# google/FluidNet

Hardware: NVIDIA H100
Metric: sim steps/sec on 128^3 MAC grid (CNN proj) (higher is better)
Workload: dtype f32

## Files before the change

### fluidnet_b200/csrc/tfl_api.cu

```cuda
#include <string.h>
#include <algorithm>
#include <cmath>
#include <string>
#include <vector>

#include "tfl_api_internal.h"

namespace {

void widen_for_forward_pass(const tfl_ctx* ctx, const Geo& g, Geo* gf) {
  if (!ctx->slab) { gf->zlo = 0; gf->zhi = g.nz; return; }
  const int lo_lim = (g.zoff == 0) ? 0 : 1;
  const int hi_lim = (g.zoff + g.nz == g.gnz) ? g.nz : g.nz - 1;
  gf->zlo = std::max(lo_lim, g.zlo - ctx->slab_margin);
  gf->zhi = std::min(hi_lim, g.zhi + ctx->slab_margin);
}

int flag_cache_ensure(tfl_ctx* ctx, const Geo& g) {
  auto& fc = ctx->fcache;
  const size_t cells = (size_t)g.n * g.nb;
  if (!fc.changed) {
    void* p = nullptr;
    TFL_CUDA(ctx, cudaMalloc(&p, sizeof(int)));
    fc.changed = (int*)p;
// ... 739 lines not shown

int tfl_debug_advect_tile(tfl_ctx* ctx, int mode, int variant) {
  if (!ctx) return 1;
  ctx->tile.mode = mode;
  ctx->tile.variant = variant;
  return 0;
}

int tfl_debug_time_advect_kernel(tfl_ctx* ctx, int on) {
  if (!ctx) return 1;
  DeviceGuard guard_(ctx);
  auto& tl = ctx->tile;
  if (on && !tl.ev0) { cudaEventCreate(&tl.ev0); cudaEventCreate(&tl.ev1); }
  tl.timed = on != 0 && tl.ev0 && tl.ev1;
  return 0;
}
float tfl_debug_last_advect_kernel_ms(tfl_ctx* ctx) {
  if (!ctx || !ctx->tile.ev0) return -1.0f;
  DeviceGuard guard_(ctx);
  float ms = -1.0f;
  if (cudaEventSynchronize(ctx->tile.ev1) != cudaSuccess || cudaEventElapsedTime(&ms, ctx->tile.ev0, ctx->tile.ev1) != cudaSuccess) {
    cudaGetLastError();
    return -1.0f;
  }
  return ms;
}

static int set_const_vals(tfl_ctx* ctx, const tfl_state* s) {
  if (s->p_bc.data && s->p_bc_inv_mask.data && tfl_apply_bc(ctx, &s->p, &s->p_bc_inv_mask, &s->p_bc)) return 1;
  if (s->U_bc.data && s->U_bc_inv_mask.data && tfl_apply_bc(ctx, &s->U, &s->U_bc_inv_mask, &s->U_bc)) return 1;
  if (s->density.data && s->density_bc.data && s->density_bc_inv_mask.data &&
      tfl_apply_bc(ctx, &s->density, &s->density_bc_inv_mask, &s->density_bc))
    return 1;
  return 0;
}

static int simulate_step_fused(tfl_ctx* ctx, const tfl_state* s, const tfl_mconf* mc, tfl_cnn* m, const Geo& g) {
  const size_t cells = (size_t)g.n * g.nb;
  const bool has_density = s->density.data != nullptr;
  if (cnn_ensure_act(ctx, m, g)) return 1;
  if (arena_reserve(ctx, carve_bytes({cells * 4, cells * 4 * g.nc, cells * 4, cells * 4 * g.nc, cells * 4 * g.nc,
                                      cells * 12, cells * 4, cells * 4, 4 * (size_t)g.nb, cells * 12, cells / 4 + 64})))
    return 1;
  Carver cv(ctx);
  float* fwd_s = cv.take<float>(cells);
  float* fwd_pos = cv.take<float>(cells * g.nc);
  float* tmp_s = cv.take<float>(cells);
  float* fwd_u = cv.take<float>(cells * g.nc);
  float* tmp_u = cv.take<float>(cells * g.nc);
  float* curl = cv.take<float>(cells * 3);
  float* cnorm = cv.take<float>(cells);
  float* p_net = cv.take<float>(cells);
  float* scale = cv.take<float>(g.nb);
  float* force = cv.take<float>(cells * 3);
  unsigned char* qmask_buf = cv.take<unsigned char>(cells / 4 + 64);
  cudaStream_t st = ctx->stream;
  unsigned char *fl8 = nullptr, *clear = nullptr;
  if (prepare_flags(ctx, s->flags.data, g, &fl8, &clear)) return 1;
  const bool ov = ctx->ov.active;
  if (ov) TFL_CUDA(ctx, cudaStreamWaitEvent(st, ctx->ev_u_in, 0));
  const unsigned char* qmask = nullptr;
  const bool u_bc0 = s->U_bc.data && s->U_bc_inv_mask.data;
  const bool d_bc0 = has_density && s->density_bc.data && s->density_bc_inv_mask.data;
  bool qmask_on_side = false;
  if (has_density) {
    TFL_CUDA(ctx, cudaEventRecord(ctx->ev_fork, st));
// ... 29 lines not shown
  const bool u_bc = s->U_bc.data && s->U_bc_inv_mask.data;
  const bool d_bc = has_density && s->density_bc.data && s->density_bc_inv_mask.data;
  float bs[3] = {0.0f, 0.0f, 0.0f};
  const int do_buoy = has_density && fo.buoyancy;
  if (do_buoy)
    for (int a = 0; a < 3; a++) bs[a] = (-fo.buoy[a]) * scale_dt;
  launch_post_advect(has_density ? tmp_s : nullptr, tmp_u, fl8, has_density ? s->density.data : nullptr,
                     s->U.data, u_bc ? s->U_bc_inv_mask.data : nullptr, u_bc ? s->U_bc.data : nullptr,
                     d_bc ? s->density_bc_inv_mask.data : nullptr, d_bc ? s->density_bc.data : nullptr, qmask, do_buoy, bs,
                     g, st);
  ctx->launches += 1;
  if (ov && has_density && ctx->ov.density_host) {
    TFL_CUDA(ctx, cudaEventRecord(ctx->ev_d_ready, st));
    TFL_CUDA(ctx, cudaStreamWaitEvent(ctx->copy_out, ctx->ev_d_ready, 0));
    TFL_CUDA(ctx, cudaMemcpyAsync(ctx->ov.density_host, s->density.data, ctx->ov.density_bytes, cudaMemcpyDeviceToHost,
                                  ctx->copy_out));
    TFL_CUDA(ctx, cudaEventRecord(ctx->ev_d_out, ctx->copy_out));
    ctx->ov.density_sent = true;
  }
  if (fo.gravity) {
    const float f[3] = {fo.grav[0] * scale_dt, fo.grav[1] * scale_dt, fo.grav[2] * scale_dt};
    launch_add_gravity(s->U.data, fl8, f, g, st);
    ctx->launches += 1;
  }
  if (fo.vorticity) {
    launch_vort_curl(s->U.data, curl, cnorm, force, fo.vort_amp, g, st);
    ctx->launches += 2;
  }
  double* sums = ctx->dscratch + 64;
  TFL_CUDA(ctx, cudaMemsetAsync(sums, 0, sizeof(double) * 2 * g.nb, st));
  launch_vort_bc_mask(s->U.data, fl8, force, fo.vorticity, u_bc ? s->U_bc_inv_mask.data : nullptr,
                      u_bc ? s->U_bc.data : nullptr, qmask, 1, sums, g, st);
  const ConvTcGeo& tg = m->act_geo;
  if (ov) TFL_CUDA(ctx, cudaStreamWaitEvent(st, ctx->ev_p_in, 0));
  launch_cnn_inputs_fused(s->p.data, s->U.data, fl8, sums, mc->normalize_input_threshold, scale, m->act[0].get(),
                          tg.px, tg.py, g, st);
  run_conv_stack(m, p_net, st);
  launch_cnn_finish_fused(p_net, s->U.data, fl8, scale, s->p.data, u_bc ? s->U_bc_inv_mask.data : nullptr,
                          u_bc ? s->U_bc.data : nullptr, qmask, -1e6f, 1e6f, g, st);
  ctx->launches += 6;
  return check_launch(ctx, "simulate_step (fused)");
}

static bool fused_step_applies(const tfl_ctx* ctx, const tfl_state* s, const tfl_mconf* mc, const tfl_cnn* cnn) {
  return mc->sim_method == TFL_SIM_CONVNET && cnn && cnn->tc_ok && cnn->mode > 0 && cnn->default_inputs && !ctx->slab &&
         s->flags.nb == 1 &&
         !s->p_bc.data && mc->advection_method >= 0 && mc->advection_method <= 5;
}

int tfl_simulate_step(tfl_ctx* ctx, const tfl_state* s, const tfl_mconf* mc, tfl_cnn* cnn) {
  DeviceGuard guard_(ctx);
  NvtxRange range_(__func__);
  if (!s || !mc) return fail(ctx, "simulate: nil state / mconf");
  if (check_scalar(ctx, &s->flags, "flags") || check_scalar(ctx, &s->p, "pDiv") || check_vel(ctx, &s->U, &s->flags))
    return 1;
  const int is3d = s->U.nc == 3;
  Geo g;
  if (make_geo(ctx, &s->flags, is3d, &g)) return 1;
  const bool has_density = s->density.data != nullptr;
  if (fused_step_applies(ctx, s, mc, cnn)) {
    if (has_density && (check_scalar(ctx, &s->density, "density") || !same_spatial(&s->density, &s->flags)))
      return fail(ctx, "Size mismatch");
    return simulate_step_fused(ctx, s, mc, cnn, g);
  }
  if (has_density && tfl_advect_scalar(ctx, mc->dt, &s->density, &s->U, &s->flags, mc->advection_method, 0,
                                       mc->maccormack_strength, nullptr))
    return 1;
  if (tfl_advect_vel(ctx, mc->dt, &s->U, &s->flags, mc->advection_method, mc->maccormack_strength, nullptr))
    return 1;
  if (set_const_vals(ctx, s)) return 1;
  const StepForces fo = step_forces(mc, g.nx, g.ny, g.gnz);
  if (has_density && fo.buoyancy && tfl_add_buoyancy(ctx, &s->U, &s->flags, &s->density, fo.buoy, mc->dt))
    return 1;
// ... 192 lines not shown
```

### fluidnet_b200/csrc/tfl_api_cnn.cu

```cuda
#include <string.h>
#include <algorithm>
#include <cmath>
#include <vector>

#include "tfl_api_internal.h"

constexpr int kMaxBanks = kMaxBankPtrs;
constexpr char kSlabTcOnly[] =
    "the z-slab projection runs on the tensor-core path only (the 3-D 'default' graph, single-bank or with banks "
    "split at stage 1 and joined at stage 3, in mode 1 or 2)";
constexpr char kSlabDilate[] =
    "the z-slab projection does not run banksType 'dilate' (dilated banks run on whole grids only)";
constexpr char kSlabBatchNorm[] =
    "the z-slab projection does not run batch normalization (addBatchNorm models run on whole grids only)";
constexpr char kSlabDefaultInputs[] =
    "the z-slab projection takes the default input block only (inputChannels pDiv, div, flags; normalizeInput with "
    "'std' of UDiv; no addPressureSkip)";

constexpr int kTailFloats = 64 + 8 + 8 + 1;

namespace {

template <typename T>
DevPtr<T> dev_alloc(size_t n) {
// ... 205 lines not shown
    org[i] = m->borg[i - 1];
    float* dst = m->bact[3 * (i - 1)].get();
    if (m->bank_dilate) {
      launch_tc_phase_copy(in[0], tg, dst, geo[i], i, m->tc_planes, st);
    } else {
      launch_tc_pyramid(in[i - 1], geo[i - 1], dst, geo[i], org[i - 1] & 1, st, m->tc_planes);
    }
    in[i] = dst;
  }
  for (int i = 0; i < nbk; i++) {
    float* o1 = i == 0 ? m->act[1].get() : m->bact[3 * (i - 1) + 1].get();
    float* o2 = i == 0 ? m->act[2].get() : m->bact[3 * (i - 1) + 2].get();
    ConvTcGeo g1 = geo[i], g2 = geo[i];
    if (!m->bank_dilate) {
      const int c_lo = ((zoff + p_lo - 1) >> i) - org[i], c_hi = ((zoff + p_hi) >> i) - org[i] + 1;
      g2.z_lo = std::max(0, c_lo);     g2.z_hi = std::min(geo[i].nz, c_hi);
      g1.z_lo = std::max(0, c_lo - 1); g1.z_hi = std::min(geo[i].nz, c_hi + 1);
    }
    launch_conv3_tc(in[i], o1, nullptr, m->wBk[split][2 * i].get(), m->b[m->conv0[0] + i].get(), nullptr,
                    m->tc_planes, 0, split, g1, st, act);
    if (m->bank_dilate && i > 0 && ((tg.nx | tg.ny | tg.nz) & ((1 << i) - 1)))
      launch_tc_phase_zero(o1, geo[i], i, tg, st);
    launch_conv3_tc(o1, o2, nullptr, m->wBk[split][2 * i + 1].get(), m->b[m->conv0[1] + i].get(), nullptr, 2, 0,
                    split, g2, st, act);
    l2[i] = o2;
  }
  ConvTcGeo g3 = tg;
  g3.z_lo = std::max(0, p_lo);
  g3.z_hi = std::min(tg.nz, p_hi);
  launch_tc_join(l2, geo, org, zoff, nbk, m->bank_add, m->part.get(), p_net, m->wBj[split], m->b[m->conv0[2]].get(),
                 m->tail.get(), split, g3, st, m->bank_dilate != 0, act);
}

void run_conv_stack(tfl_cnn* m, float* p_net, cudaStream_t st, int p_lo, int p_hi) {
  if (p_hi < 0) p_hi = m->act_geo.nz;
  if (m->nbanks > 1) {
    run_conv_stack_banked(m, p_net, st, p_lo, p_hi);
    return;
  }
  const ConvTcGeo& tg = m->act_geo;
  const int split = m->mode == 2 ? 1 : 0;
  ConvTcGeo g1 = tg, g2 = tg, g3 = tg;
  g3.z_lo = std::max(0, p_lo);     g3.z_hi = std::min(tg.nz, p_hi);
  g2.z_lo = std::max(0, p_lo - 1); g2.z_hi = std::min(tg.nz, p_hi + 1);
  g1.z_lo = std::max(0, p_lo - 2); g1.z_hi = std::min(tg.nz, p_hi + 2);
  TcEpi e1, e2, e3;
  e1.relu6 = e2.relu6 = e3.relu6 = m->nonlin == 3;
  if (m->bn && !m->bn_batch) {
    e1.ac = m->bn_ac[0].get();
    e2.ac = m->bn_ac[1].get();
  }
  float *a0 = m->act[0].get(), *a1 = m->act[1].get(), *a2 = m->act[2].get(), *tail = m->tail.get();
  const float *w1 = m->wBk[split][0].get(), *w2 = m->wBk[split][1].get(), *w3 = m->wBj[split][0].get();
  if (!m->bn_batch) {
    launch_conv3_tc(a0, a1, nullptr, w1, m->b[0].get(), nullptr, m->tc_planes, 0, split, g1, st, e1);
    launch_conv3_tc(a1, a2, nullptr, w2, m->b[1].get(), nullptr, 2, 0, split, g2, st, e2);
    launch_conv3_tc(a2, nullptr, p_net, w3, m->b[2].get(), tail, 2, 1, split, g3, st, e3);
    return;
  }
  double* part = m->bn_part.get();
  float* ac = m->bn_tcac.get();
  const long long count = (long long)tg.nb * tg.nz * tg.ny * tg.nx;
  auto stats = [&](const float* buf, int l) {
    launch_tc_bn_stats(buf, tg, part, st);
    const float* wb = m->bn_wb[l].get();
    launch_bn_finalize(part, 8, count, wb, wb + 8, m->bn_eps[l], ac + 16 * l, nullptr, st);
  };
  launch_conv3_tc(a0, a1, nullptr, w1, m->b[0].get(), nullptr, m->tc_planes, 0, split, tg, st, e1);
  stats(a1, 0);
  launch_tc_bn_apply(a1, tg, ac, st);
  launch_conv3_tc(a1, a2, nullptr, w2, m->b[1].get(), nullptr, 2, 0, split, tg, st, e2);
  stats(a2, 1);
  launch_tc_bn_apply(a2, tg, ac + 16, st);
  launch_conv3_tc(a2, a1, nullptr, w3, m->b[2].get(), nullptr, 2, 0, split, tg, st, e3);
  stats(a1, 2);
  launch_tc_bn_tail(a1, tg, ac + 32, tail, e3.relu6, 0, part, nullptr, nullptr, st);
  launch_bn_finalize(part, 8, count, m->bn_wb[3].get(), m->bn_wb[3].get() + 8, m->bn_eps[3], ac + 48, nullptr, st);
  launch_tc_bn_tail(a1, tg, ac + 32, tail, e3.relu6, 1, nullptr, ac + 48, p_net, st);
}

static const tfl_cnn_inputs kDefaultInputs = {1, 0, 1, 1, 0, 0, 0};

namespace {

struct CnnSpec {
  int is_3d, n_layers;
  const int32_t *cin, *cout, *ksize, *pool, *up;
  int pool_is_max, nonlin_sigmoid;
// ... 960 lines not shown
```

### fluidnet_b200/csrc/tfl_api_internal.h

```cpp
#pragma once
#include <cuda_runtime.h>
#include <stdarg.h>
#include <stdio.h>
#include <nvtx3/nvToolsExt.h>
#include <nccl.h>
#include <initializer_list>
#include <memory>
#include <string>
#include <vector>

#include "tfl_kernels.h"
#include "tfl_cnn_tc.h"

using namespace tfl;

struct CudaFree {
  void operator()(void* p) const { cudaFree(p); }
};
template <typename T>
using DevPtr = std::unique_ptr<T, CudaFree>;

constexpr char kConvZStalled[] =
    "internal error, the z-streaming tensor-core convolution's pipeline stalled (a bounded wait ran out)";

// ... 169 lines not shown
  if (U->nc != 2 && U->nc != 3) return fail(ctx, "2D velocity field must have only 2 channels");
  if (U->nc == 2 && flags->nz != 1) return fail(ctx, "2D velocity field but zdepth > 1");
  if (!same_spatial(U, flags)) return fail(ctx, "Size mismatch");
  return 0;
}

inline int make_geo(tfl_ctx* ctx, const tfl_grid* flags, int is3d, Geo* g) {
  g->nx = flags->nx; g->ny = flags->ny; g->nz = flags->nz; g->nb = flags->nb;
  g->is3d = is3d ? 1 : 0;
  g->nc = is3d ? 3 : 2;
  g->n = (long long)flags->nx * flags->ny * flags->nz;
  g->faults = ctx->counters;
  if (ctx->slab) {
    if (!is3d) return fail(ctx, "slab decomposition needs a 3D grid");
    g->zoff = ctx->zoff; g->gnz = ctx->gnz; g->zlo = ctx->zlo; g->zhi = ctx->zhi;
    if (g->zlo < 0 || g->zhi > g->nz || g->zlo >= g->zhi || g->zoff < 0 || g->zoff + g->nz > g->gnz)
      return fail(ctx, "slab range does not fit the local grid");
  } else {
    g->zoff = 0; g->gnz = flags->nz; g->zlo = 0; g->zhi = flags->nz;
  }
  if (!is3d && flags->nz != 1) return fail(ctx, "2D grid must have zsize == 1");
  if (g->n >= (1LL << 31) || g->n * (long long)g->nb * 3 >= (1LL << 31) * 4) return fail(ctx, "grid too large");
  return 0;
}

struct StepForces {
  bool buoyancy, gravity, vorticity;
  float buoy[3], grav[3];
  float vort_amp;
};
StepForces step_forces(const tfl_mconf* mc, int nx, int ny, int gnz);

int cnn_ensure_act(tfl_ctx* ctx, tfl_cnn* m, const Geo& g);
void run_conv_stack(tfl_cnn* m, float* p_net, cudaStream_t st, int p_lo = 0, int p_hi = -1);
int cnn_slab_check(tfl_ctx* ctx, const tfl_cnn* m, int margin, int gnz, int ny, int nx, int zoff, int nz, int own_lo,
                   int own_hi);
```

### fluidnet_b200/csrc/tfl_cnn_tc.cu

```cuda
#include <cuda_runtime.h>
#include <stdint.h>

#include "tfl_cnn_tc.h"

namespace tfl {

namespace {

constexpr int kTX = 32;
constexpr int kGroups = 9;
constexpr int kThreads = 256;
constexpr int kDPitch = 24;

template <bool SPLIT> struct Tile {
  static constexpr int TY = SPLIT ? 4 : 8;
  static constexpr int TZ = SPLIT ? 5 : 6;
  static constexpr int PY = TY + 2, PZ = TZ + 2;
  static constexpr int RB = TY / 2;
  static constexpr int POS = kTX * PY * PZ;
  static constexpr int PLANE_BYTES = POS * 16;
  static constexpr int MTILES = TZ * RB;
};

template <int IN_PLANES, bool SPLIT> struct Layout {
  using T = Tile<SPLIT>;
  static constexpr int NB = SPLIT ? 48 : 32;
  static constexpr int GROUPS = IN_PLANES == 1 ? 5 : kGroups;
  static constexpr int ZERO_BYTES = IN_PLANES == 1 ? 64 * 16 : 0;
  static constexpr int PSTRIDE = T::PLANE_BYTES + ZERO_BYTES;
  static constexpr int LO_OFF = IN_PLANES * PSTRIDE;
  static constexpr int A_BYTES = (SPLIT ? 2 : 1) * LO_OFF;
  static constexpr int B_GROUP_BYTES = 2 * NB * 16;
  static constexpr int B_BYTES = GROUPS * B_GROUP_BYTES;
  static constexpr int BYTES = A_BYTES + B_BYTES + 2 * 64 * kDPitch * 4 + 4 * 96;
};

constexpr int kZWarpGroups = 4;
constexpr int kZThreads = 128 * (kZWarpGroups + 1);
constexpr int kWWMax = 128;
constexpr int kZLaunchRegs = 96;
template <bool SPLIT> struct ZRegs {
  static constexpr int PRODUCER = SPLIT ? 64 : 128;
  static constexpr int CONSUMER = SPLIT ? 104 : 88;
  static_assert(128 * PRODUCER + 128 * kZWarpGroups * CONSUMER <= kZThreads * kZLaunchRegs, "register file");
};
constexpr long long kZSpinCycles = 1ll << 31;

template <int IN_PLANES, bool SPLIT> struct ZLayout {
  static constexpr int TY = SPLIT ? 4 : 8;
  static constexpr int PY = TY + 2;
  static constexpr int NB = SPLIT ? 48 : 32;
  static constexpr int GROUPS = IN_PLANES == 1 ? 5 : kGroups;
  static constexpr int ZERO_BYTES = IN_PLANES == 1 ? 64 * 16 : 0;
  static constexpr int B_GROUP_BYTES = 2 * NB * 16;
  static constexpr int B_BYTES = GROUPS * B_GROUP_BYTES;
  static constexpr int SLOT_CHUNKS = SPLIT ? 4 : 2;
  static constexpr size_t bytes(int ww) {
    return (size_t)3 * SLOT_CHUNKS * PY * ww * 16 + ZERO_BYTES + B_BYTES + (size_t)kZWarpGroups * ww * kDPitch * 4 +
           4 * 96 + 64;
  }
};

struct ZSched {
  int ww;
  int nty;
  int zc, nzc;
  int items;
};

__host__ __device__ constexpr int layer1_dz(int gi) { return gi < 3 ? -1 : 1; }
__host__ __device__ constexpr int layer1_dy(int gi) { return gi < 3 ? gi - 1 : (gi == 3 ? -1 : 1); }

__device__ __forceinline__ uint32_t smem_u32(const void* p) {
  return (uint32_t)__cvta_generic_to_shared(p);
}
__device__ __forceinline__ void cp_async16(uint32_t dst, const void* src) {
// ... 87 lines not shown
  for (int o = 0; o < 4; o++) h[o] = tc_act(h[o], ep.relu6);
  if constexpr (!FINAL) {
    if (ep.ac) {
#pragma unroll
      for (int o = 0; o < 4; o++) h[o] = fmaf(sTail[8 + 4 * half + o], h[o], sTail[16 + 4 * half + o]);
    }
    if (valid) out[out_idx + half * plane_g] = make_float4(h[0], h[1], h[2], h[3]);
  } else {
    float hh[8];
#pragma unroll
    for (int o = 0; o < 4; o++) {
      const float other = __shfl_xor_sync(0xffffffffu, h[o], 1);
      hh[o] = half ? other : h[o];
      hh[4 + o] = half ? h[o] : other;
    }
    const float* w4 = sTail + 8 + 32 * half;
    const float* b4 = sTail + 8 + 64 + 4 * half;
    const float* w5 = sTail + 8 + 64 + 8 + 4 * half;
    const float b5 = sTail[8 + 64 + 8 + 8];
    float part = 0.0f;
#pragma unroll
    for (int o = 0; o < 4; o++) {
      float a = b4[o];
#pragma unroll
      for (int c = 0; c < 8; c++) a = fmaf(hh[c], w4[o * 8 + c], a);
      a = tc_act(a, ep.relu6);
      part = fmaf(a, w5[o], part);
    }
    const float pacc = b5 + (part + __shfl_xor_sync(0xffffffffu, part, 1));
    if (valid && half == 0) p_net[p_idx] = pacc;
  }
}

template <int IN_PLANES, bool FINAL, bool SPLIT>
__global__ void __launch_bounds__(kZThreads, 1)
k_conv3_tc_z(const float4* __restrict__ in, float4* __restrict__ out, float* __restrict__ p_net,
             const float* __restrict__ wB, const float* __restrict__ bias, const float* __restrict__ tail,
             ConvTcGeo g, ZSched s, TcEpi ep) {
  extern __shared__ __align__(1024) uint8_t smem[];
  using L = ZLayout<IN_PLANES, SPLIT>;
  using R = ZRegs<SPLIT>;
  constexpr int TY = L::TY, PY = L::PY;
  const int ww = s.ww, ntile = ww >> 6;
  const int gbytes = PY * ww * 16;
  const int lo_off = 2 * gbytes;
  const int slot_bytes = L::SLOT_CHUNKS * gbytes;
  uint8_t* sRing = smem;
  uint8_t* sZero = smem + 3 * slot_bytes;
  uint8_t* sB = sZero + L::ZERO_BYTES;
  float* sD = (float*)(sB + L::B_BYTES);
  float* sTail = sD + kZWarpGroups * ww * kDPitch;
  uint64_t* sBar = (uint64_t*)(sTail + 96);
  volatile int* sAbort = (volatile int*)(sBar + 6);

  const int tid = threadIdx.x, warp = tid >> 5, lane = tid & 31;

  const uint32_t bar_u = smem_u32(sBar);
  auto setup = [&]() {
    for (int i = tid; i < L::ZERO_BYTES / 16; i += kZThreads) ((float4*)sZero)[i] = make_float4(0.f, 0.f, 0.f, 0.f);
#pragma unroll 1
    for (int i = tid; i < L::B_BYTES / 16; i += kZThreads) ((float4*)sB)[i] = __ldg((const float4*)wB + i);
    const int n_tail = FINAL ? (8 + 64 + 8 + 8 + 1) : 8;
    for (int i = tid; i < n_tail; i += kZThreads) sTail[i] = (i < 8) ? bias[i] : tail[i - 8];
    if (!FINAL && ep.ac && tid < 16) sTail[8 + tid] = ep.ac[tid];
    if (tid == 0) {
      for (int k = 0; k < 3; k++) {
        mbar_init(bar_u + 8 * k, 1);
        mbar_init(bar_u + 24 + 8 * k, kZWarpGroups);
      }
      *sAbort = 0;
    }
    asm volatile("fence.proxy.async.shared::cta;" ::: "memory");
    __syncthreads();
  };

  const long long plane_g = (long long)(g.nz + 2) * g.py * g.px;
  const long long batch_g = plane_g * 2;
  const int npos = PY * ww;
  const int wg = warp >> 2, wq = warp & 3;
  const int tw = tid & 127;
  auto item_geo = [&](int item, int& y0, int& za, int& zb, int& b) {
    const int ty = item % s.nty, zc = (item / s.nty) % s.nzc;
    b = item / s.nty / s.nzc;
    y0 = ty * TY;
    za = g.z_lo + zc * s.zc;
    zb = min(za + s.zc, g.z_hi);
  };

  if (wg == kZWarpGroups) {
    if constexpr (R::PRODUCER < kZLaunchRegs) asm volatile("setmaxnreg.dec.sync.aligned.u32 %0;" ::"n"(R::PRODUCER));
    if constexpr (R::PRODUCER > kZLaunchRegs) asm volatile("setmaxnreg.inc.sync.aligned.u32 %0;" ::"n"(R::PRODUCER));
    setup();
    constexpr int PER = (PY * kWWMax + 127) / 128;
    float4 v[PER][IN_PLANES];
    auto load = [&](int y0, int b, int pz) {
      const float4* inb = in + b * batch_g;
#pragma unroll
      for (int it = 0; it < PER; it++) {
        const int idx = tw + it * 128;
        const int row = idx / ww, gx = 1 + idx - row * ww, gy = y0 + row;
        const bool inside = idx < npos && gx < g.px && gy < g.py;
        const long long go = inside ? ((long long)pz * g.py + gy) * g.px + gx : 0;
#pragma unroll
        for (int h = 0; h < IN_PLANES; h++) v[it][h] = __ldg(inb + h * plane_g + go);
      }
    };
    int item = blockIdx.x, y0, za, zb, b;
    if (item < s.items) {
      item_geo(item, y0, za, zb, b);
      load(y0, b, za);
    }
    for (int q = 0, pz = za; item < s.items; q++) {
      const int slot = q % 3;
      auto put = [&](uint8_t* slot_p, int c) {
#pragma unroll
        for (int it = 0; it < PER; it++) {
          const int idx = tw + it * 128;
          if (idx < npos) {
            const float4 w = v[it][IN_PLANES == 2 ? c : 0];
            uint8_t* dst = slot_p + c * gbytes + idx * 16;
            if constexpr (SPLIT) {
              const float4 hi = tf32_hi(w);
              *(float4*)dst = hi;
              *(float4*)(dst + lo_off) = make_float4(w.x - hi.x, w.y - hi.y, w.z - hi.z, w.w - hi.w);
            } else {
              *(float4*)dst = w;
            }
          }
        }
      };
      if (IN_PLANES == 1 && pz > za) put(sRing + ((q + 2) % 3) * slot_bytes, 1);
      if (q >= 3) mbar_wait(bar_u + 24 + 8 * slot, ((q / 3) - 1) & 1, sAbort);
      put(sRing + slot * slot_bytes, 0);
      if (IN_PLANES == 2) put(sRing + slot * slot_bytes, 1);
      asm volatile("fence.proxy.async.shared::cta;" ::: "memory");
      wg_barrier(1 + kZWarpGroups);
      if (tw == 0) mbar_arrive(bar_u + 8 * slot);
      if (++pz > zb + 1) {
        item += gridDim.x;
        if (item >= s.items) break;
        item_geo(item, y0, za, zb, b);
        pz = za;
      }
      load(y0, b, pz);
    }
  } else {
    if constexpr (R::CONSUMER > kZLaunchRegs) asm volatile("setmaxnreg.inc.sync.aligned.u32 %0;" ::"n"(R::CONSUMER));
    if constexpr (R::CONSUMER < kZLaunchRegs) asm volatile("setmaxnreg.dec.sync.aligned.u32 %0;" ::"n"(R::CONSUMER));
    long long* dbg = g_tc_dbg;
    if (dbg && tid == 0) dbg[blockIdx.x * 8 + 0] = clock64();
    setup();
    const uint32_t sRing_u = smem_u32(sRing), sB_u = smem_u32(sB), sZero_u = smem_u32(sZero);
    float* myD = sD + wg * ww * kDPitch;
    const int half = tw & 1;
    const float* bs = sTail + 4 * half;
    int qa = 0;
    int waited = 0;
    auto wait_plane = [&](int q) {
      for (; waited <= q; waited++) mbar_wait(bar_u + 8 * (waited % 3), (waited / 3) & 1, sAbort);
    };
    auto release_plane = [&](int q) {
      if (tw == 0) mbar_arrive(bar_u + 24 + 8 * (q % 3));
    };
    for (int item = blockIdx.x; item < s.items; item += gridDim.x) {
      int y0, za, zb, b;
      item_geo(item, y0, za, zb, b);
      const bool has_rows = y0 + wg < g.ny;

      for (int z = za; z < zb; z++) {
        const int qz = qa + (z - za);
        uint32_t base[3];
#pragma unroll
        for (int d = 0; d < 3; d++) base[d] = sRing_u + (uint32_t)(((qz + d) % 3) * slot_bytes);
        wait_plane(qz + 1);
        if (dbg && tid == 0 && item == blockIdx.x && z == za) dbg[blockIdx.x * 8 + 1] = clock64();
        if (!has_rows) {
          wait_plane(qz + 2);
// ... 359 lines not shown
  }
  const int ntz = (g.z_hi - g.z_lo + T::TZ - 1) / T::TZ;
  ConvTcGeo gg = g;
  gg.ntz = ntz;
  gg.nty = (g.ny + T::TY - 1) / T::TY;
  dim3 grid(g.ntx, gg.nty, ntz * g.nb);
  kern<<<grid, kThreads, smem, st>>>(in, out, p_net, wB, bias, tail, gg, js, ep);
}

ZSched z_schedule(const ConvTcGeo& g, int ty, int nsm) {
  ZSched s;
  s.zc = 1;
  s.ww = g.nx > 64 ? kWWMax : 64;
  s.nty = (g.ny + ty - 1) / ty;
  const long long cols = (long long)g.nb * s.nty;
  const int nzo = g.z_hi - g.z_lo;
  long long best = -1;
  for (int zc = 1; zc <= nzo; zc++) {
    const long long items = cols * ((nzo + zc - 1) / zc);
    const long long grid = items < nsm ? items : nsm;
    const long long cost = (items + grid - 1) / grid * (zc + 2);
    if (best < 0 || cost <= best) {
      best = cost;
      s.zc = zc;
    }
  }
  s.nzc = (nzo + s.zc - 1) / s.zc;
  s.items = (int)(cols * s.nzc);
  return s;
}

int g_z_grid_cap = 0;

template <int IN_PLANES, bool FINAL, bool SPLIT>
void launch_z(const float4* in, float4* out, float* p_net, const float* wB, const float* bias, const float* tail,
              const ConvTcGeo& g, cudaStream_t st, const TcEpi& ep) {
  using L = ZLayout<IN_PLANES, SPLIT>;
  if (g.z_hi <= g.z_lo || g.nb < 1 || g.ny < 1 || g.nx < 1) return;
  auto kern = k_conv3_tc_z<IN_PLANES, FINAL, SPLIT>;
  static unsigned long long configured = 0;
  int dev = 0, nsm = 0;
  cudaGetDevice(&dev);
  if (!((configured >> (dev & 63)) & 1ULL)) {
    cudaFuncSetAttribute(kern, cudaFuncAttributeMaxDynamicSharedMemorySize, (int)L::bytes(kWWMax));
    configured |= 1ULL << (dev & 63);
  }
  cudaDeviceGetAttribute(&nsm, cudaDevAttrMultiProcessorCount, dev);
  const ZSched s = z_schedule(g, L::TY, nsm);
  int grid = s.items < nsm ? s.items : nsm;
  if (g_z_grid_cap > 0 && grid > g_z_grid_cap) grid = g_z_grid_cap;
  kern<<<grid, kZThreads, L::bytes(s.ww), st>>>(in, out, p_net, wB, bias, tail, g, s, ep);
}

__global__ void k_tc_pyramid(const float4* __restrict__ in, ConvTcGeo gi, float4* __restrict__ out, ConvTcGeo go,
                             int z_phase, int planes, long long total) {
  const long long t = (long long)blockIdx.x * blockDim.x + threadIdx.x;
  if (t >= total) return;
  const int nzr = go.z_hi - go.z_lo;
  const int x = (int)(t % go.nx), y = (int)((t / go.nx) % go.ny);
  const int z = go.z_lo + (int)((t / ((long long)go.nx * go.ny)) % nzr);
  const long long b = t / ((long long)go.nx * go.ny * nzr);
  const long long iplane = (long long)(gi.nz + 2) * gi.py * gi.px, oplane = (long long)(go.nz + 2) * go.py * go.px;
  for (int q = 0; q < planes; q++) {
    const float4* ib = in + (b * 2 + q) * iplane;
    float sx = 0.0f, sy = 0.0f, sz = 0.0f, sw = 0.0f;
    for (int dz = 0; dz < 2; dz++)
      for (int dy = 0; dy < 2; dy++)
        for (int dx = 0; dx < 2; dx++) {
          const float4 v =
              __ldg(ib + ((long long)(2 * z + z_phase + dz + 1) * gi.py + (2 * y + dy + 1)) * gi.px + (2 * x + dx + 1));
          sx += v.x; sy += v.y; sz += v.z; sw += v.w;
        }
    out[(b * 2 + q) * oplane + ((long long)(z + 1) * go.py + (y + 1)) * go.px + (x + 1)] =
        make_float4(sx / 8.0f, sy / 8.0f, sz / 8.0f, planes == 2 ? sw / 8.0f : 0.0f);
  }
}

__device__ __forceinline__ bool phase_voxel(long long t, const ConvTcGeo& gs, int sh, const ConvTcGeo& gf, long long* e,
                                            int* sx, int* sy, int* sz, long long* b, int* x, int* y, int* z) {
  *sx = (int)(t % gs.nx);
  *sy = (int)((t / gs.nx) % gs.ny);
  *sz = (int)((t / ((long long)gs.nx * gs.ny)) % gs.nz);
  *e = t / ((long long)gs.nx * gs.ny * gs.nz);
  const int m = (1 << sh) - 1;
// ... 121 lines not shown
            union { float f; uint32_t u; } hi;
            hi.f = v;
            if (split) hi.u &= 0xFFFFE000u;
            const int n = kx * 8 + o, kc = kc0 + (c >> 2);
            blk[(kc * NB + n) * 4 + (c & 3)] = hi.f;
            if (split) blk[(kc * NB + 24 + n) * 4 + (c & 3)] = v - hi.f;
          }
    }
}

int launch_conv3_tc_join(const TcJoinSrc& src, float* p_net, const float* wB, const float* bias, const float* tail,
                         int split, const ConvTcGeo& g, cudaStream_t st, const TcEpi& ep) {
  if (src.n < 1 || src.n > kTcMaxBanks) return -1;
  if (split) launch_one<2, true, true, true>(nullptr, nullptr, p_net, wB, bias, tail, g, st, src, ep);
  else launch_one<2, true, false, true>(nullptr, nullptr, p_net, wB, bias, tail, g, st, src, ep);
  return 1;
}

void launch_tc_pyramid(const float* in, const ConvTcGeo& gin, float* out, const ConvTcGeo& gout, int z_phase,
                       cudaStream_t st, int planes) {
  const long long total = (long long)gout.nb * (gout.z_hi - gout.z_lo) * gout.ny * gout.nx;
  if (total <= 0) return;
  k_tc_pyramid<<<(unsigned)((total + 255) / 256), 256, 0, st>>>((const float4*)in, gin, (float4*)out, gout, z_phase,
                                                                 planes, total);
}

int launch_conv3_tc(const float* in, float* out, float* p_net, const float* wB, const float* bias,
                    const float* tail, int in_planes, int final_layer, int split, const ConvTcGeo& g,
                    cudaStream_t st, const TcEpi& ep) {
  const float4* i4 = (const float4*)in;
  float4* o4 = (float4*)out;
#define TFL_TC_CASE(P, F, S)                                                   \
  if (in_planes == P && (final_layer != 0) == F && (split != 0) == S) {        \
    if (g.nx <= kWWMax) launch_z<P, F, S>(i4, o4, p_net, wB, bias, tail, g, st, ep); \
    else launch_one<P, F, S>(i4, o4, p_net, wB, bias, tail, g, st, TcJoinSrc{}, ep); \
    return 1;                                                                  \
  }
  TFL_TC_CASE(1, false, false) TFL_TC_CASE(2, false, false) TFL_TC_CASE(2, true, false)
  TFL_TC_CASE(1, false, true) TFL_TC_CASE(2, false, true) TFL_TC_CASE(2, true, true)
#undef TFL_TC_CASE
  return -1;
}

}
```

### fluidnet_b200/csrc/tfl_cnn_tc.h

```cpp
#pragma once
#include <cuda_runtime.h>
#include <stddef.h>

namespace tfl {

struct ConvTcGeo {
  int nb, nz, ny, nx;
  int px, py;
  int ntx, nty, ntz;
  int z_lo, z_hi;
};

ConvTcGeo make_conv_tc_geo(int nb, int nz, int ny, int nx);
size_t conv_tc_act_bytes(const ConvTcGeo& g);
int conv_tc_b_floats(int split);
void conv_tc_set_debug(long long* dev_buf);
void conv_tc_set_z_grid(int ctas);
int conv_tc_take_z_fault(cudaStream_t st);
void conv_tc_pack_weights(const float* w , int cin, int split, float* out);
struct TcEpi {
  const float* ac = nullptr;
  int relu6 = 0;
};
int launch_conv3_tc(const float* in, float* out, float* p_net, const float* wB, const float* bias,
                    const float* tail, int in_planes, int final_layer, int split, const ConvTcGeo& g,
                    cudaStream_t st, const TcEpi& ep = TcEpi());

constexpr int kTcMaxBanks = 8;
struct TcJoinSrc {
  const float* p[kTcMaxBanks];
  int px[kTcMaxBanks], py[kTcMaxBanks], nz[kTcMaxBanks], shift[kTcMaxBanks], org[kTcMaxBanks];
  int phase[kTcMaxBanks];
  int zoff;
  int n;
  int part_mode;
  float* partial;
};
int launch_conv3_tc_join(const TcJoinSrc& src, float* p_net, const float* wB, const float* bias, const float* tail,
                         int split, const ConvTcGeo& g, cudaStream_t st, const TcEpi& ep = TcEpi());

void launch_tc_bn_stats(const float* buf, const ConvTcGeo& g, double* part, cudaStream_t st);
void launch_tc_bn_apply(float* buf, const ConvTcGeo& g, const float* ac, cudaStream_t st);
void launch_tc_bn_tail(const float* buf, const ConvTcGeo& g, const float* ac3, const float* tail, int relu6,
                       int pass_b, double* part, const float* ac4, float* p_net, cudaStream_t st);
void launch_tc_pyramid(const float* in, const ConvTcGeo& gin, float* out, const ConvTcGeo& gout, int z_phase,
                       cudaStream_t st, int planes = 1);

ConvTcGeo make_conv_tc_phase_geo(int nb, int nz, int ny, int nx, int sh);
void launch_tc_phase_copy(const float* in, const ConvTcGeo& gfull, float* out, const ConvTcGeo& gsub, int sh,
                          int planes, cudaStream_t st);
void launch_tc_phase_zero(float* buf, const ConvTcGeo& gsub, int sh, const ConvTcGeo& gfull, cudaStream_t st);
void launch_tc_phase_gather(const float* in, const ConvTcGeo& gsub, float* out, const ConvTcGeo& gfull, int sh,
                            cudaStream_t st);

}
```

### fluidnet_b200/csrc/tfl_device.cuh

```cuda
#pragma once
#include <cuda_runtime.h>
#include <stdint.h>
#include <float.h>

namespace tfl {

struct Geo {
  int nx, ny, nz;
  int gnz;
  int zoff;
  int zlo, zhi;
  int nb;
  int is3d;
  int nc;
  long long n;
  unsigned long long* faults;
};

struct V3 { float x, y, z; };

template <bool IS3D>
__device__ __forceinline__ Geo static_geo(const Geo& gin) {
  Geo g = gin;
  g.is3d = IS3D ? 1 : 0;
// ... 386 lines not shown
    if ((j > 0 && (flag_i(fl, g, k, j - 1, i) & kStick)) ||
        (j < g.ny - 1 && (flag_i(fl, g, k, j + 1, i) & kStick))) { z[0] = true; if (g.is3d) z[2] = true; }
    if (g.is3d && ((kg > 0 && (flag_i(fl, g, local_z(g, kg - 1), j, i) & kStick)) ||
                   (kg < g.gnz - 1 && (flag_i(fl, g, local_z(g, kg + 1), j, i) & kStick)))) {
      z[0] = true; z[1] = true;
    }
  }
}


__device__ __forceinline__ V3 conf_force(const float* __restrict__ cb, const float* __restrict__ cn,
                                         const Geo& g, int k, int j, int i, float strength) {
  if (on_border(g, k, j, i)) return V3{0.0f, 0.0f, 0.0f};
  const int c = cell(g, k, j, i);
  const int sy = g.nx, sz = g.nx * g.ny;
  V3 gr = {0.0f, 0.0f, 0.0f};
  gr.x = 0.5f * (__ldg(cn + c + 1) - __ldg(cn + c - 1));
  gr.y = 0.5f * (__ldg(cn + c + sy) - __ldg(cn + c - sy));
  if (g.is3d) gr.z = 0.5f * (__ldg(cn + c + sz) - __ldg(cn + c - sz));
  const float gn = norm3(gr);
  if (gn > 1e-6f) { gr.x /= gn; gr.y /= gn; gr.z /= gn; } else { gr.x = gr.y = gr.z = 0.0f; }
  const V3 w = {__ldg(cb + c), __ldg(cb + g.n + c), __ldg(cb + 2 * g.n + c)};
  V3 f;
  f.x = ((gr.y * w.z) - (gr.z * w.y)) * strength;
  f.y = ((gr.z * w.x) - (gr.x * w.z)) * strength;
  f.z = ((gr.x * w.y) - (gr.y * w.x)) * strength;
  return f;
}


__device__ __forceinline__ float scale_from_sums(const double* __restrict__ sums, int b, long long n,
                                                 float threshold) {
  const float sum = (float)sums[2 * b], sumsq = (float)sums[2 * b + 1];
  float out = sumsq * (float)n;
  out = out + (-1.0f) * (sum * sum);
  out = out / (float)((double)n * (double)(n - 1));
  out = sqrtf(out);
  return (out < threshold) ? threshold : out;
}

__device__ __forceinline__ void block_accumulate(double s, double ss, double* __restrict__ dst) {
  __shared__ double sh[2][32];
  const int tid = (threadIdx.z * blockDim.y + threadIdx.y) * blockDim.x + threadIdx.x;
  const int lane = tid & 31, w = tid >> 5;
  for (int o = 16; o > 0; o >>= 1) {
    s += __shfl_down_sync(0xffffffffu, s, o);
    ss += __shfl_down_sync(0xffffffffu, ss, o);
  }
  if (lane == 0) { sh[0][w] = s; sh[1][w] = ss; }
  __syncthreads();
  if (w == 0) {
    const int nw = (blockDim.x * blockDim.y * blockDim.z + 31) >> 5;
    s = lane < nw ? sh[0][lane] : 0.0;
    ss = lane < nw ? sh[1][lane] : 0.0;
    for (int o = 16; o > 0; o >>= 1) {
      s += __shfl_down_sync(0xffffffffu, s, o);
      ss += __shfl_down_sync(0xffffffffu, ss, o);
    }
    if (lane == 0) {
      atomicAdd(dst, s);
      atomicAdd(dst + 1, ss);
    }
  }
}

}
```

Measured before the change: 1149.

## Fuse CNN input construction into the first tensor-core conv layer's producer

Adds an INPUTS variant of the warp-specialized z-streaming conv kernel. Its producer warps read pressure, velocity and flags directly, compute divergence, normalise by the std scale and write the scale out, instead of running a separate input-building kernel that materialises the padded activation buffer. The producer loop is restructured to prefetch the next item's raw inputs before the current tile is published, and register splits are rebalanced for this variant. This removes one launch and one full-grid write/read round trip. In exchange the producer does more work per tile and has less register headroom, which could stall the MMA consumers.

After: 1167 (median of 6 runs). 1.6% higher.

```diff
diff --git a/fluidnet_b200/csrc/tfl_api.cu b/fluidnet_b200/csrc/tfl_api.cu
--- a/fluidnet_b200/csrc/tfl_api.cu
+++ b/fluidnet_b200/csrc/tfl_api.cu
@@ -795,6 +795,13 @@
   if (s->density.data && s->density_bc.data && s->density_bc_inv_mask.data &&
       tfl_apply_bc(ctx, &s->density, &s->density_bc_inv_mask, &s->density_bc))
     return 1;
+  return 0;
+}
+
+static bool g_force_input_pass = false;
+
+int tfl_debug_cnn_input_pass(int force) {
+  g_force_input_pass = force != 0;
   return 0;
 }
 
@@ -890,13 +897,19 @@
   launch_vort_bc_mask(s->U.data, fl8, force, fo.vorticity, u_bc ? s->U_bc_inv_mask.data : nullptr,
                       u_bc ? s->U_bc.data : nullptr, qmask, 1, sums, g, st);
   const ConvTcGeo& tg = m->act_geo;
+  const bool inputs_in_conv =
+      m->nbanks == 1 && !m->bn_batch && conv_tc_inputs_apply(tg, m->mode == 2) && !g_force_input_pass;
+  const TcIn in1{s->p.data, s->U.data, fl8, sums, mc->normalize_input_threshold, scale};
   if (ov) TFL_CUDA(ctx, cudaStreamWaitEvent(st, ctx->ev_p_in, 0));
-  launch_cnn_inputs_fused(s->p.data, s->U.data, fl8, sums, mc->normalize_input_threshold, scale, m->act[0].get(),
-                          tg.px, tg.py, g, st);
-  run_conv_stack(m, p_net, st);
+  if (!inputs_in_conv) {
+    launch_cnn_inputs_fused(s->p.data, s->U.data, fl8, sums, mc->normalize_input_threshold, scale, m->act[0].get(),
+                            tg.px, tg.py, g, st);
+    ctx->launches += 1;
+  }
+  run_conv_stack(m, p_net, st, 0, -1, inputs_in_conv ? &in1 : nullptr);
   launch_cnn_finish_fused(p_net, s->U.data, fl8, scale, s->p.data, u_bc ? s->U_bc_inv_mask.data : nullptr,
                           u_bc ? s->U_bc.data : nullptr, qmask, -1e6f, 1e6f, g, st);
-  ctx->launches += 6;
+  ctx->launches += 5;
   return check_launch(ctx, "simulate_step (fused)");
 }
 
diff --git a/fluidnet_b200/csrc/tfl_api_cnn.cu b/fluidnet_b200/csrc/tfl_api_cnn.cu
--- a/fluidnet_b200/csrc/tfl_api_cnn.cu
+++ b/fluidnet_b200/csrc/tfl_api_cnn.cu
@@ -261,7 +261,7 @@
                  m->tail.get(), split, g3, st, m->bank_dilate != 0, act);
 }
 
-void run_conv_stack(tfl_cnn* m, float* p_net, cudaStream_t st, int p_lo, int p_hi) {
+void run_conv_stack(tfl_cnn* m, float* p_net, cudaStream_t st, int p_lo, int p_hi, const TcIn* in1) {
   if (p_hi < 0) p_hi = m->act_geo.nz;
   if (m->nbanks > 1) {
     run_conv_stack_banked(m, p_net, st, p_lo, p_hi);
@@ -282,7 +282,8 @@
   float *a0 = m->act[0].get(), *a1 = m->act[1].get(), *a2 = m->act[2].get(), *tail = m->tail.get();
   const float *w1 = m->wBk[split][0].get(), *w2 = m->wBk[split][1].get(), *w3 = m->wBj[split][0].get();
   if (!m->bn_batch) {
-    launch_conv3_tc(a0, a1, nullptr, w1, m->b[0].get(), nullptr, m->tc_planes, 0, split, g1, st, e1);
+    if (in1) launch_conv3_tc_inputs(*in1, a1, w1, m->b[0].get(), split, g1, st, e1);
+    else launch_conv3_tc(a0, a1, nullptr, w1, m->b[0].get(), nullptr, m->tc_planes, 0, split, g1, st, e1);
     launch_conv3_tc(a1, a2, nullptr, w2, m->b[1].get(), nullptr, 2, 0, split, g2, st, e2);
     launch_conv3_tc(a2, nullptr, p_net, w3, m->b[2].get(), tail, 2, 1, split, g3, st, e3);
     return;
diff --git a/fluidnet_b200/csrc/tfl_api_internal.h b/fluidnet_b200/csrc/tfl_api_internal.h
--- a/fluidnet_b200/csrc/tfl_api_internal.h
+++ b/fluidnet_b200/csrc/tfl_api_internal.h
@@ -225,6 +225,6 @@
 StepForces step_forces(const tfl_mconf* mc, int nx, int ny, int gnz);
 
 int cnn_ensure_act(tfl_ctx* ctx, tfl_cnn* m, const Geo& g);
-void run_conv_stack(tfl_cnn* m, float* p_net, cudaStream_t st, int p_lo = 0, int p_hi = -1);
+void run_conv_stack(tfl_cnn* m, float* p_net, cudaStream_t st, int p_lo = 0, int p_hi = -1, const TcIn* in1 = nullptr);
 int cnn_slab_check(tfl_ctx* ctx, const tfl_cnn* m, int margin, int gnz, int ny, int nx, int zoff, int nz, int own_lo,
                    int own_hi);
diff --git a/fluidnet_b200/csrc/tfl_cnn_tc.cu b/fluidnet_b200/csrc/tfl_cnn_tc.cu
--- a/fluidnet_b200/csrc/tfl_cnn_tc.cu
+++ b/fluidnet_b200/csrc/tfl_cnn_tc.cu
@@ -2,6 +2,7 @@
 #include <stdint.h>
 
 #include "tfl_cnn_tc.h"
+#include "tfl_device.cuh"
 
 namespace tfl {
 
@@ -39,9 +40,9 @@
 constexpr int kZThreads = 128 * (kZWarpGroups + 1);
 constexpr int kWWMax = 128;
 constexpr int kZLaunchRegs = 96;
-template <bool SPLIT> struct ZRegs {
-  static constexpr int PRODUCER = SPLIT ? 64 : 128;
-  static constexpr int CONSUMER = SPLIT ? 104 : 88;
+template <bool SPLIT, bool INPUTS = false> struct ZRegs {
+  static constexpr int PRODUCER = INPUTS ? 96 : SPLIT ? 64 : 128;
+  static constexpr int CONSUMER = INPUTS ? 96 : SPLIT ? 104 : 88;
   static_assert(128 * PRODUCER + 128 * kZWarpGroups * CONSUMER <= kZThreads * kZLaunchRegs, "register file");
 };
 constexpr long long kZSpinCycles = 1ll << 31;
@@ -195,14 +196,15 @@
   }
 }
 
-template <int IN_PLANES, bool FINAL, bool SPLIT>
+template <int IN_PLANES, bool FINAL, bool SPLIT, bool INPUTS = false>
 __global__ void __launch_bounds__(kZThreads, 1)
 k_conv3_tc_z(const float4* __restrict__ in, float4* __restrict__ out, float* __restrict__ p_net,
              const float* __restrict__ wB, const float* __restrict__ bias, const float* __restrict__ tail,
-             ConvTcGeo g, ZSched s, TcEpi ep) {
+             ConvTcGeo g, ZSched s, TcEpi ep, TcIn ti) {
+  static_assert(!INPUTS || (IN_PLANES == 1 && !FINAL && SPLIT), "the network input is layer 1's, in 3xTF32");
   extern __shared__ __align__(1024) uint8_t smem[];
   using L = ZLayout<IN_PLANES, SPLIT>;
-  using R = ZRegs<SPLIT>;
+  using R = ZRegs<SPLIT, INPUTS>;
   constexpr int TY = L::TY, PY = L::PY;
   const int ww = s.ww, ntile = ww >> 6;
   const int gbytes = PY * ww * 16;
@@ -256,25 +258,89 @@
     setup();
     constexpr int PER = (PY * kWWMax + 127) / 128;
     float4 v[PER][IN_PLANES];
+    constexpr int RAW = INPUTS ? PER : 1;
+    int r_f[RAW];
+    float r_pd[RAW], r_u[RAW][6];
+    float sc = 1.0f;
     auto load = [&](int y0, int b, int pz) {
-      const float4* inb = in + b * batch_g;
-#pragma unroll
-      for (int it = 0; it < PER; it++) {
-        const int idx = tw + it * 128;
-        const int row = idx / ww, gx = 1 + idx - row * ww, gy = y0 + row;
-        const bool inside = idx < npos && gx < g.px && gy < g.py;
-        const long long go = inside ? ((long long)pz * g.py + gy) * g.px + gx : 0;
-#pragma unroll
-        for (int h = 0; h < IN_PLANES; h++) v[it][h] = __ldg(inb + h * plane_g + go);
+      if constexpr (INPUTS) {
+        const long long n = (long long)g.nz * g.ny * g.nx;
+        const float* pdb = ti.p_div + b * n;
+        const float* ub = ti.U + b * 3 * n;
+        const unsigned char* fb = ti.flags + b * n;
+        const int k = pz - 1;
+#pragma unroll
+        for (int it = 0; it < PER; it++) {
+          const int idx = tw + it * 128;
+          const int row = idx / ww, i = idx - row * ww, j = y0 + row - 1;
+          const bool inside = idx < npos && i < g.nx && j >= 0 && j < g.ny && k >= 0 && k < g.nz;
+          const bool interior = inside && i >= 1 && i <= g.nx - 2 && j >= 1 && j <= g.ny - 2 && k >= 1 && k <= g.nz - 2;
+          const int c = inside ? (k * g.ny + j) * g.nx + i : 0;
+          r_f[it] = inside ? (int)__ldg(fb + c) : -1;
+          r_pd[it] = inside ? __ldg(pdb + c) : 0.0f;
+          r_u[it][0] = interior ? __ldg(ub + c) : 0.0f;
+          r_u[it][1] = interior ? __ldg(ub + c + 1) : 0.0f;
+          r_u[it][2] = interior ? __ldg(ub + n + c) : 0.0f;
+          r_u[it][3] = interior ? __ldg(ub + n + c + g.nx) : 0.0f;
+          r_u[it][4] = interior ? __ldg(ub + 2 * n + c) : 0.0f;
+          r_u[it][5] = interior ? __ldg(ub + 2 * n + c + g.nx * g.ny) : 0.0f;
+        }
+      } else {
+        const float4* inb = in + b * batch_g;
+#pragma unroll
+        for (int it = 0; it < PER; it++) {
+          const int idx = tw + it * 128;
+          const int row = idx / ww, gx = 1 + idx - row * ww, gy = y0 + row;
+          const bool inside = idx < npos && gx < g.px && gy < g.py;
+          const long long go = inside ? ((long long)pz * g.py + gy) * g.px + gx : 0;
+#pragma unroll
+          for (int h = 0; h < IN_PLANES; h++) v[it][h] = __ldg(inb + h * plane_g + go);
+        }
+      }
+    };
+    auto build_inputs = [&]() {
+      if constexpr (INPUTS) {
+#pragma unroll
+        for (int it = 0; it < PER; it++) {
+          const int f = r_f[it];
+          float dv = 0.0f;
+          if (f & kFluid) {
+            dv = r_u[it][0] - r_u[it][1] + r_u[it][2] - r_u[it][3];
+            dv += (r_u[it][4] - r_u[it][5]);
+          }
+          v[it][0] = f < 0 ? make_float4(0.f, 0.f, 0.f, 0.f)
+                           : make_float4(r_pd[it] / sc, dv / sc,
+                                         (f == kFluid) ? 0.0f : ((f == kObstacle) ? 1.0f : -1.0f), 0.0f);
+        }
+      }
+    };
+    auto item_scale = [&](int y0, int za, int b) {
+      if constexpr (INPUTS) {
+        sc = scale_from_sums(ti.sums, b, 3 * (long long)g.nz * g.ny * g.nx, ti.threshold);
+        if (tw == 0 && y0 == 0 && za == g.z_lo) ti.scale_out[b] = sc;
       }
     };
     int item = blockIdx.x, y0, za, zb, b;
     if (item < s.items) {
       item_geo(item, y0, za, zb, b);
+      item_scale(y0, za, b);
       load(y0, b, za);
     }
     for (int q = 0, pz = za; item < s.items; q++) {
       const int slot = q % 3;
+      build_inputs();
+      int nitem = item, npz = pz + 1, ny0 = y0, nza = za, nzb = zb, nb = b;
+      if (npz > zb + 1) {
+        nitem += gridDim.x;
+        if (nitem < s.items) {
+          item_geo(nitem, ny0, nza, nzb, nb);
+          npz = nza;
+        }
+      }
+      if (INPUTS && nitem < s.items) {
+        if (nitem != item) item_scale(ny0, nza, nb);
+        load(ny0, nb, npz);
+      }
       auto put = [&](uint8_t* slot_p, int c) {
 #pragma unroll
         for (int it = 0; it < PER; it++) {
@@ -299,13 +365,8 @@
       asm volatile("fence.proxy.async.shared::cta;" ::: "memory");
       wg_barrier(1 + kZWarpGroups);
       if (tw == 0) mbar_arrive(bar_u + 8 * slot);
-      if (++pz > zb + 1) {
-        item += gridDim.x;
-        if (item >= s.items) break;
-        item_geo(item, y0, za, zb, b);
-        pz = za;
-      }
-      load(y0, b, pz);
+      if (!INPUTS && nitem < s.items) load(ny0, nb, npz);
+      item = nitem; pz = npz; y0 = ny0; za = nza; zb = nzb; b = nb;
     }
   } else {
     if constexpr (R::CONSUMER > kZLaunchRegs) asm volatile("setmaxnreg.inc.sync.aligned.u32 %0;" ::"n"(R::CONSUMER));
@@ -731,12 +792,12 @@
 
 int g_z_grid_cap = 0;
 
-template <int IN_PLANES, bool FINAL, bool SPLIT>
+template <int IN_PLANES, bool FINAL, bool SPLIT, bool INPUTS = false>
 void launch_z(const float4* in, float4* out, float* p_net, const float* wB, const float* bias, const float* tail,
-              const ConvTcGeo& g, cudaStream_t st, const TcEpi& ep) {
+              const ConvTcGeo& g, cudaStream_t st, const TcEpi& ep, const TcIn& ti = TcIn{}) {
   using L = ZLayout<IN_PLANES, SPLIT>;
   if (g.z_hi <= g.z_lo || g.nb < 1 || g.ny < 1 || g.nx < 1) return;
-  auto kern = k_conv3_tc_z<IN_PLANES, FINAL, SPLIT>;
+  auto kern = k_conv3_tc_z<IN_PLANES, FINAL, SPLIT, INPUTS>;
   static unsigned long long configured = 0;
   int dev = 0, nsm = 0;
   cudaGetDevice(&dev);
@@ -748,7 +809,7 @@
   const ZSched s = z_schedule(g, L::TY, nsm);
   int grid = s.items < nsm ? s.items : nsm;
   if (g_z_grid_cap > 0 && grid > g_z_grid_cap) grid = g_z_grid_cap;
-  kern<<<grid, kZThreads, L::bytes(s.ww), st>>>(in, out, p_net, wB, bias, tail, g, s, ep);
+  kern<<<grid, kZThreads, L::bytes(s.ww), st>>>(in, out, p_net, wB, bias, tail, g, s, ep, ti);
 }
 
 __global__ void k_tc_pyramid(const float4* __restrict__ in, ConvTcGeo gi, float4* __restrict__ out, ConvTcGeo go,
@@ -936,7 +997,7 @@
   float4* o4 = (float4*)out;
 #define TFL_TC_CASE(P, F, S)                                                   \
   if (in_planes == P && (final_layer != 0) == F && (split != 0) == S) {        \
-    if (g.nx <= kWWMax) launch_z<P, F, S>(i4, o4, p_net, wB, bias, tail, g, st, ep); \
+    if (conv_tc_streams(g)) launch_z<P, F, S>(i4, o4, p_net, wB, bias, tail, g, st, ep); \
     else launch_one<P, F, S>(i4, o4, p_net, wB, bias, tail, g, st, TcJoinSrc{}, ep); \
     return 1;                                                                  \
   }
@@ -946,4 +1007,14 @@
   return -1;
 }
 
-}
+bool conv_tc_streams(const ConvTcGeo& g) { return g.nx <= kWWMax; }
+bool conv_tc_inputs_apply(const ConvTcGeo& g, int split) { return split && conv_tc_streams(g); }
+
+int launch_conv3_tc_inputs(const TcIn& in, float* out, const float* wB, const float* bias, int split,
+                           const ConvTcGeo& g, cudaStream_t st, const TcEpi& ep) {
+  if (!conv_tc_inputs_apply(g, split)) return -1;
+  launch_z<1, false, true, true>(nullptr, (float4*)out, nullptr, wB, bias, nullptr, g, st, ep, in);
+  return 1;
+}
+
+}
diff --git a/fluidnet_b200/csrc/tfl_cnn_tc.h b/fluidnet_b200/csrc/tfl_cnn_tc.h
--- a/fluidnet_b200/csrc/tfl_cnn_tc.h
+++ b/fluidnet_b200/csrc/tfl_cnn_tc.h
@@ -25,6 +25,18 @@
 int launch_conv3_tc(const float* in, float* out, float* p_net, const float* wB, const float* bias,
                     const float* tail, int in_planes, int final_layer, int split, const ConvTcGeo& g,
                     cudaStream_t st, const TcEpi& ep = TcEpi());
+bool conv_tc_streams(const ConvTcGeo& g);
+struct TcIn {
+  const float* p_div;
+  const float* U;
+  const unsigned char* flags;
+  const double* sums;
+  float threshold;
+  float* scale_out;
+};
+bool conv_tc_inputs_apply(const ConvTcGeo& g, int split);
+int launch_conv3_tc_inputs(const TcIn& in, float* out, const float* wB, const float* bias, int split,
+                           const ConvTcGeo& g, cudaStream_t st, const TcEpi& ep = TcEpi());
 
 constexpr int kTcMaxBanks = 8;
 struct TcJoinSrc {
diff --git a/fluidnet_b200/csrc/tfl_device.cuh b/fluidnet_b200/csrc/tfl_device.cuh
--- a/fluidnet_b200/csrc/tfl_device.cuh
+++ b/fluidnet_b200/csrc/tfl_device.cuh
@@ -442,9 +442,9 @@
 __device__ __forceinline__ float scale_from_sums(const double* __restrict__ sums, int b, long long n,
                                                  float threshold) {
   const float sum = (float)sums[2 * b], sumsq = (float)sums[2 * b + 1];
-  float out = sumsq * (float)n;
-  out = out + (-1.0f) * (sum * sum);
-  out = out / (float)((double)n * (double)(n - 1));
+  float out = __fmul_rn(sumsq, (float)n);
+  out = __fadd_rn(out, __fmul_rn(-1.0f, __fmul_rn(sum, sum)));
+  out = __fdiv_rn(out, (float)((double)n * (double)(n - 1)));
   out = sqrtf(out);
   return (out < threshold) ? threshold : out;
 }
```
